# yshen47/SGAM_NeurIPS22

Hardware: AMD Instinct MI355X
Metric: generated RGB-D frames/sec (256x256, GoogleEarth) (higher is better)
Workload: dtype f32; 1 GPU; GoogleEarth-Infinite 256x256 inference loop (BASELINE configs[2]): forward-splat warp (N<=3) + VQGAN encode/quantise(4096)/decode + frame feedback, in-HBM frame store; frames_per_gpu=1110, scenes=1, parallelism=scene-parallel x1, launch=hip-graph replay of the VQGAN forward, f32_products=exact hi/lo fp16 split on the fp16 matrix cores, fp32 accumulate

## Files before the change

sgam_neurips22_amd/csrc/conv_f32x.hip:

```cpp
#include <type_traits>

#include "sgam_common.h"

namespace {

constexpr int XGN_MAXC = 1024;

typedef unsigned int u32x4 __attribute__((ext_vector_type(4)));
typedef unsigned int u32x2 __attribute__((ext_vector_type(2)));
typedef _Float16 f16x8 __attribute__((ext_vector_type(8)));

struct XParams {
    const float *x, *bias, *res;
    const unsigned short *w;
    float *out, *ws;
    int B, Hi, Wi, Cin, Ho, Wo, N, KH, KW, stride, pad_t, pad_l, ups;
    int lda, ldb, ldc, ldr, n_valid, bias_per_row;
    int M, ksplit, iters_total, iters_per_split;
    int gx, gy, xcd_swizzle;
    unsigned x_bytes, w_plane_bytes;
    const float *gn_stats, *gn_gamma, *gn_beta;
    int gn_swish;
    const double *gn_partial_in;
    double gn_inv_n;
// ... 120 lines not shown
                                           rb, (int)xsel(n < n_lim, (unsigned)n * 4u, OOB), 0, 0));
#pragma unroll
            for (int e = 0; e < 16; ++e)
                region[(i * 32 + (e & 3) + 8 * (e >> 2) + row_h) * LDR + j * 32 + col_l] = acc[i][j][e] * inv + bias_n;
        }
    constexpr int C4 = WN / 4;
    constexpr int RPP = 64 / C4;
    const int c4 = lane % C4, rr0 = lane / C4;
    const int n4 = wn0 + c4 * 4;
    const bool n_ok = n4 < n_lim;
    float gs = 0.f, gss = 0.f;
    bool bad = false;
#pragma unroll
    for (int pass = 0; pass < WM / RPP; ++pass) {
        const int row = rr0 + pass * RPP;
        const int m = rowmap(wm * (BM / WGM) + row);
        const bool ok = n_ok && m < p.M;
        f32x4 v = *reinterpret_cast<const f32x4 *>(region + row * LDR + c4 * 4);
        const f32x4 rv = __builtin_bit_cast(f32x4, __builtin_amdgcn_raw_buffer_load_b128(
                                                       rr, (int)xsel(ok, (unsigned)(m * p.ldr + n4) * 4u, OOB), 0, 0));
        if (p.bias_per_row) {
            const float bm = __builtin_bit_cast(float, __builtin_amdgcn_raw_buffer_load_b32(
                                                           rb, (int)xsel(ok, (unsigned)m * 4u, OOB), 0, 0));
            v += bm;
        }
        v += rv;
        __builtin_amdgcn_raw_buffer_store_b128(__builtin_bit_cast(u32x4, v), ro, (int)xsel(ok, (unsigned)(m * ldo + n4) * 4u, OOB), 0, 0);
        if (ok) {
            const float t4 = (v[0] + v[1]) + (v[2] + v[3]);
            gs += t4;
            gss += (v[0] * v[0] + v[1] * v[1]) + (v[2] * v[2] + v[3] * v[3]);
            bad |= sgam_not_finite(t4);
        }
    }
    if (bad && !to_ws && p.range_flag) atomicOr(p.range_flag, 1);
    if (p.gn_partial && !to_ws) {
        float *sl = region;
        sl[lane * 2] = gs;
        sl[lane * 2 + 1] = gss;
        const int c4_per_group = p.gn_cpg / 4;
        const int groups_here = C4 / c4_per_group;
        if (lane < groups_here) {
            double ds = 0.0, dss = 0.0;
            for (int r = 0; r < RPP; ++r)
                for (int k = 0; k < c4_per_group; ++k) {
                    const int l = r * C4 + lane * c4_per_group + k;
                    ds += (double)sl[l * 2];
                    dss += (double)sl[l * 2 + 1];
                }
            const int g = (wn0 / p.gn_cpg) + lane;
            const int groups = p.N / p.gn_cpg;
            if (g < groups) {
                const int chunk = bx * 2 + wm;
                const int hw = p.Ho * p.Wo;
                const int b = (bx * BM) / hw;
                const int chunks_per_b = ((hw + BM - 1) / BM) * 2;
                const int cb = chunk - b * chunks_per_b;
                double *o = p.gn_partial + (((int64_t)b * chunks_per_b + cb) * groups + g) * 2;
                o[0] = ds;
                o[1] = dss;
                if (WGM == 1) {
                    o[groups * 2] = 0.0;
                    o[groups * 2 + 1] = 0.0;
                }
            }
        }
    }
}

template <int BM, int BN, bool UPS, bool ASCALE>
__global__ __launch_bounds__(256 * wk_of(BM, BN)) void conv_gemm_f32x_kernel(const XParams p) {
    constexpr int XBK = xbk_of(BM, BN), WK = wk_of(BM, BN), NT = 256 * WK;
    constexpr int XLD = XBK + 8;
    constexpr int TM = BM / 64, TN = BN / 64;
    constexpr int PF = (BM * BN >= 128 * 128) ? 1 : 2;
    constexpr int AC = XBK / 4;
    static_assert(NT / AC == 32, "the A staging map assumes 32 rows per pass");
    constexpr int AR = BM / 32;
    constexpr int SL = XBK / 32;
    constexpr int NPB = (BN / 32) * SL * 256 / NT;
    constexpr int KS = XBK / 16;
    static_assert(KS % WK == 0, "k-steps split evenly over the wavefront groups");
    constexpr int PLANE_A = BM * XLD, PLANE_B = BN * XLD;
    constexpr int STAGE = 2 * PLANE_A + 2 * PLANE_B;
    __shared__ __attribute__((aligned(16))) unsigned short smem[2 * STAGE];

    const int tid = threadIdx.x;
    const int lane = tid & 63;
    const int wave = (tid >> 6) & 3;
    const int wk = tid >> 8;
    const int wm = wave >> 1, wn = wave & 1;
    int bx, by, bz;
    xcd_block(p, bx, by, bz);
    const int m0 = bx * BM;
    const int n0 = by * BN;

    const __amdgpu_buffer_rsrc_t rx = __builtin_amdgcn_make_buffer_rsrc((void *)p.x, 0, (int)p.x_bytes, 0x00020000);
    const __amdgpu_buffer_rsrc_t rw = __builtin_amdgcn_make_buffer_rsrc((void *)p.w, 0, (int)p.w_plane_bytes, 0x00020000);

    const int it0 = bz * p.iters_per_split;
    const int it1 = min(p.iters_total, it0 + p.iters_per_split);

    const int col4 = tid % AC;
    const int row_in_pass = tid / AC;
    const int Hl = p.ups ? 2 * p.Hi : p.Hi;
    const int Wl = p.ups ? 2 * p.Wi : p.Wi;

    int a_iy0[AR], a_ix0[AR], a_base[AR];
    unsigned a_rowoff[AR], a_tapmask[AR];
#pragma unroll
    for (int r = 0; r < AR; ++r) {
        const int m = m0 + row_in_pass + 32 * r;
        const bool ok = m < p.M;
        const int mm = ok ? m : 0;
        const int hw = p.Ho * p.Wo;
        const int b = mm / hw;
        const int rem = mm - b * hw;
        const int oy = rem / p.Wo;
        const int ox = rem - oy * p.Wo;
        a_iy0[r] = ok ? oy * p.stride - p.pad_t : -(1 << 28);
        a_ix0[r] = ox * p.stride - p.pad_l;
        a_base[r] = b * p.Hi * p.Wi;
        a_rowoff[r] = (unsigned)((a_base[r] + a_iy0[r] * p.Wi + a_ix0[r]) * p.lda + col4 * 4) * 4u;
        unsigned mk = 0;
        for (int t = 0; t < p.KH * p.KW; ++t) {
            const int iy = a_iy0[r] + t / p.KW, ix = a_ix0[r] + t % p.KW;
            mk |= (((unsigned)iy < (unsigned)p.Hi && (unsigned)ix < (unsigned)p.Wi) ? 1u : 0u) << t;
        }
        a_tapmask[r] = mk;
    }
    unsigned b_off[NPB];
    int b_lds[NPB], b_k[NPB];
    const unsigned slabs_per_row = (unsigned)p.ldb / 32u;
#pragma unroll
    for (int j = 0; j < NPB; ++j) {
        const int L = tid + NT * j, blk = L >> 8, pi = L & 255;
        const int nt = blk / SL, sl = blk - nt * SL;
        const int plane = pi >> 7, kk = (pi >> 6) & 1, kh = (pi >> 5) & 1, row = pi & 31;
        const int n = n0 + nt * 32 + row;
        b_off[j] = n < p.N ? ((((unsigned)(n >> 5) * slabs_per_row + (unsigned)sl) * 256u + (unsigned)pi) * 16u) : 0xC0000000u;
        b_lds[j] = plane * PLANE_B + (nt * 32 + row) * XLD + sl * 32 + kk * 16 + kh * 8;
        b_k[j] = sl * 32 + kk * 16 + kh * 8;
    }

    const int taps = p.KH * p.KW;
    int ch = it0 / taps;
    int tap = it0 - ch * taps;
    int ky = tap / p.KW;
    int kx = tap - ky * p.KW;

    f32x4 areg[PF][AR];
    u32x4 bp[PF][NPB];
    auto issue_loads = [&](const int st, bool live) {
        const int coff = ch * XBK + col4 * 4;
        const bool k_ok = live && coff < p.Cin;
        if constexpr (UPS) {
#pragma unroll
            for (int r = 0; r < AR; ++r) {
                const int iy = a_iy0[r] + ky, ix = a_ix0[r] + kx;
                const bool ok = k_ok && (unsigned)iy < (unsigned)Hl && (unsigned)ix < (unsigned)Wl;
                const int py = iy >> 1, px = ix >> 1;
                const unsigned off = (unsigned)((a_base[r] + py * p.Wi + px) * p.lda + coff) * 4u;
                areg[st][r] = __builtin_bit_cast(f32x4, __builtin_amdgcn_raw_buffer_load_b128(rx, (int)xsel(ok, off, p.x_bytes), 0, 0));
            }
        } else {
            const unsigned tap_off = (unsigned)((ky * p.Wi + kx) * p.lda + ch * XBK) * 4u;
#pragma unroll
            for (int r = 0; r < AR; ++r) {
                const bool ok = k_ok && ((a_tapmask[r] >> tap) & 1u);
                areg[st][r] = __builtin_bit_cast(f32x4, __builtin_amdgcn_raw_buffer_load_b128(
                                                            rx, (int)xsel(ok, a_rowoff[r] + tap_off, p.x_bytes), 0, 0));
            }
        }
        const unsigned koff = (unsigned)(tap * p.Cin + ch * XBK) * 128u;
#pragma unroll
        for (int j = 0; j < NPB; ++j) {
            const bool kb_ok = live && (ch * XBK + b_k[j]) < p.Cin;
            bp[st][j] = __builtin_amdgcn_raw_buffer_load_b128(rw, (int)xsel(kb_ok, b_off[j] + koff, p.w_plane_bytes), 0, 0);
        }
        ++tap;
        if (++kx == p.KW) {
            kx = 0;
            ++ky;
        }
        if (tap == taps) {
            tap = 0; ky = 0; kx = 0;
            ++ch;
        }
    };
    auto store_lds = [&](const int st, int buf) {
        unsigned short *ah = smem + buf * STAGE;
        unsigned short *al = ah + PLANE_A;
        unsigned short *bhp = al + PLANE_A;
#pragma unroll
        for (int r = 0; r < AR; ++r) {
            u32x2 hi, lo;
            split4(ASCALE ? areg[st][r] * p.a_scale : areg[st][r], hi, lo);
            const int o = (row_in_pass + 32 * r) * XLD + col4 * 4;
            *reinterpret_cast<u32x2 *>(ah + o) = hi;
            *reinterpret_cast<u32x2 *>(al + o) = lo;
        }
#pragma unroll
        for (int j = 0; j < NPB; ++j) *reinterpret_cast<u32x4 *>(bhp + b_lds[j]) = bp[st][j];
    };

    constexpr bool SEPACC = (TM * TN == 1);
    f32x16 acc[TM][TN], accs[1];
#pragma unroll
    for (int i = 0; i < TM; ++i)
#pragma unroll
        for (int j = 0; j < TN; ++j)
#pragma unroll
            for (int e = 0; e < 16; ++e) acc[i][j][e] = 0.f;
#pragma unroll
    for (int e = 0; e < 16; ++e) accs[0][e] = 0.f;

    const int frag_row = lane & 31;
    const int frag_k = (lane >> 5) * 8;

#pragma unroll
    for (int s = 0; s < PF; ++s) issue_loads(s, it0 + s < it1);
    store_lds(0, 0);
    issue_loads(0, it0 + PF < it1);
    __syncthreads();

    int it = it0;
    while (it < it1) {
#pragma unroll
        for (int s = 0; s < PF; ++s) {
            if (it < it1) {
                const int nst = (s + 1) % PF;
                const int buf = (it - it0) & 1;
                const unsigned short *ah = smem + buf * STAGE + (wm * (BM / 2) + frag_row) * XLD + frag_k;
                const unsigned short *al = ah + PLANE_A;
                const unsigned short *bhp = smem + buf * STAGE + 2 * PLANE_A + (wn * (BN / 2) + frag_row) * XLD + frag_k;
                const unsigned short *blp = bhp + PLANE_B;
#pragma unroll
                for (int kq = 0; kq < KS / WK; ++kq) {
                    const int kk = kq * WK + wk;
                    if (kq == (KS / WK) / 2) {
                        store_lds(nst, buf ^ 1);
                        issue_loads(nst, it + 1 + PF < it1);
                        __builtin_amdgcn_sched_barrier(0);
                    }
                    u32x4 fah[TM], fal[TM], fbh[TN], fbl[TN];
#pragma unroll
                    for (int i = 0; i < TM; ++i) {
                        fah[i] = *reinterpret_cast<const u32x4 *>(ah + i * 32 * XLD + kk * 16);
                        fal[i] = *reinterpret_cast<const u32x4 *>(al + i * 32 * XLD + kk * 16);
                    }
#pragma unroll
                    for (int j = 0; j < TN; ++j) {
                        fbh[j] = *reinterpret_cast<const u32x4 *>(bhp + j * 32 * XLD + kk * 16);
                        fbl[j] = *reinterpret_cast<const u32x4 *>(blp + j * 32 * XLD + kk * 16);
                    }
#pragma unroll
                    for (int i = 0; i < TM; ++i)
#pragma unroll
                        for (int j = 0; j < TN; ++j) {
                            if constexpr (SEPACC) {
                                accs[0] = mfma16(fal[i], fbh[j], accs[0]);
                                acc[i][j] = mfma16(fah[i], fbh[j], acc[i][j]);
                                accs[0] = mfma16(fah[i], fbl[j], accs[0]);
                            } else {
                                acc[i][j] = mfma16(fal[i], fbh[j], acc[i][j]);
                                acc[i][j] = mfma16(fah[i], fbl[j], acc[i][j]);
                                acc[i][j] = mfma16(fah[i], fbh[j], acc[i][j]);
                            }
                        }
                }
                __syncthreads();
                ++it;
            }
        }
    }

    if constexpr (SEPACC) acc[0][0] += accs[0];
    constexpr int WM = 32 * TM, WN = 32 * TN, LDR = WN + 4;
    static_assert(4 * WM * LDR * 4 <= 2 * STAGE * 2, "epilogue staging must fit the operand LDS");
    if constexpr (WK > 1) {
        constexpr int XCH = 4 * WM * LDR;
        static_assert((XCH + 4 * TM * TN * 1024) * 4 <= 2 * STAGE * 2, "k-group exchange must fit the operand LDS");
        float *xch = reinterpret_cast<float *>(smem) + XCH + wave * (TM * TN * 1024);
        if (wk == 1) {
#pragma unroll
            for (int i = 0; i < TM; ++i)
#pragma unroll
                for (int j = 0; j < TN; ++j)
#pragma unroll
                    for (int e = 0; e < 16; ++e) xch[((i * TN + j) * 16 + e) * 64 + lane] = acc[i][j][e];
        }
        __syncthreads();
        if (wk == 1) return;
#pragma unroll
        for (int i = 0; i < TM; ++i)
#pragma unroll
            for (int j = 0; j < TN; ++j)
#pragma unroll
                for (int e = 0; e < 16; ++e) acc[i][j][e] += xch[((i * TN + j) * 16 + e) * 64 + lane];
    }
    xepilogue<BM, BN, 2>(p, acc, reinterpret_cast<float *>(smem), wave, lane, bx, bz, n0, [&](int row) { return m0 + row; });
}

template <int BM, int BN, bool GN, bool UPS = false, bool GNF = false, int NB = 3>
__global__ __launch_bounds__(256, (BM == 64 && !GNF) ? XLB64 : 2) void conv3x3_f32x_halo2_kernel(const XParams p) {
    static_assert(!GNF || GN, "GNF = GroupNorm statistics folded from the producer's chunk partials: a GN kernel");
    constexpr int WGM_ = BN == 32 ? 4 : (BN == 64 ? 2 : 1), WGN_ = 4 / WGM_;
    constexpr int TH = 8, TW = BM / 8, TWS = (TW == 16) ? 4 : 3;
    constexpr int HROWS = UPS ? TH / 2 + 2 : TH + 2, HWID = UPS ? TW / 2 + 2 : TW + 2, HR = HROWS * HWID;
    static_assert(!(UPS && GN), "no GroupNorm precedes an upsampling conv");
    static_assert(BM == 128 || BM == 64, "8 x 16 or 8 x 8 output patches");
    constexpr int XBK = 32, XLD = XBK + 8;
    constexpr int TM = BM / (32 * WGM_), TN = BN / (32 * WGN_);
    constexpr int LP = UPS ? ((TW == 16) ? 408 : 240) : ((TW == 16) ? 768 : 448);
    constexpr int HPL = HROWS * LP;
    constexpr int HBUF = 2 * HPL;
    constexpr int NH = (HR * 8 + 255) / 256;
    constexpr int OP_BYTES = 2 * HBUF * 2;
    constexpr int EPI_BYTES = 4 * (32 * TM) * (32 * TN + 4) * 4;
    constexpr int TAB_BYTES = (GN && !GNF) ? XGN_MAXC * 8 : 0;
    constexpr int SM_BYTES = (OP_BYTES + TAB_BYTES) > EPI_BYTES ? (OP_BYTES + TAB_BYTES) : EPI_BYTES;
    __shared__ __attribute__((aligned(16))) unsigned short smem[SM_BYTES / 2];
    float *gn_tab = reinterpret_cast<float *>(smem + OP_BYTES / 2);

    const int tid = threadIdx.x;
    const int lane = tid & 63;
    const int wave = tid >> 6;
    const int wm = WGM_ == 4 ? wave : (WGM_ == 2 ? wave >> 1 : 0), wn = WGM_ == 4 ? 0 : (WGM_ == 2 ? (wave & 1) : wave);
    int bx, by, bz;
    xcd_block(p, bx, by, bz);
    const int n0 = by * BN;
    const int tiles_x = p.Wo / TW, tiles_img = tiles_x * (p.Ho / TH);
    const int b = bx / tiles_img;
    const int t_img = bx - b * tiles_img;
    const int ty0 = (t_img / tiles_x) * TH, tx0 = (t_img % tiles_x) * TW;

    const __amdgpu_buffer_rsrc_t rx = __builtin_amdgcn_make_buffer_rsrc((void *)p.x, 0, (int)p.x_bytes, 0x00020000);
    const __amdgpu_buffer_rsrc_t rw = __builtin_amdgcn_make_buffer_rsrc((void *)p.w, 0, (int)p.w_plane_bytes, 0x00020000);

    const int it0 = bz * p.iters_per_split;
    const int it1 = min(p.iters_total, it0 + p.iters_per_split);

    unsigned h_off[NH];
    int h_lds[NH];
#pragma unroll
    for (int j = 0; j < NH; ++j) {
        const int idx = tid + 256 * j;
        const int row = idx >> 3, col4 = idx & 7;
        const int hy = row / HWID, hx = row - hy * HWID;
        const int iy = (UPS ? ty0 / 2 : ty0) + hy - 1, ix = (UPS ? tx0 / 2 : tx0) + hx - 1;
        const bool ok = row < HR && (unsigned)iy < (unsigned)p.Hi && (unsigned)ix < (unsigned)p.Wi;
        h_off[j] = ok ? (unsigned)(((b * p.Hi + iy) * p.Wi + ix) * p.lda + col4 * 4) * 4u : 0xFFFFFFFFu;
        h_lds[j] = row < HR ? hy * LP + hx * XLD + col4 * 4 : -1;
    }
    unsigned bf_off[TN];
#pragma unroll
    for (int j = 0; j < TN; ++j) {
        const int nt = (n0 + wn * (BN / WGN_) + j * 32) >> 5;
        bf_off[j] = ((unsigned)nt * ((unsigned)p.ldb / 32u) * 256u + (unsigned)lane) * 16u;
    }

    f32x4 hreg[NH];
    f32x4 gt0, gt1;
    auto hload_issue = [&](int ch, bool live) {
        const unsigned coff = (unsigned)ch * (XBK * 4u);
#pragma unroll
        for (int j = 0; j < NH; ++j)
            hreg[j] = __builtin_bit_cast(f32x4, __builtin_amdgcn_raw_buffer_load_b128(rx, (int)(live ? h_off[j] : 0xFFFFFFFFu), (int)coff, 0));
    };
    auto hparams = [&](int ch, bool live) {
        if constexpr (GN && GNF) {
            gn_scale_shift<GNF>(p, b, (live ? ch : 0) * XBK + (tid & 7) * 4, gt0, gt1);
        } else if constexpr (GN) {
            const float *t = gn_tab + 2 * ((live ? ch : 0) * XBK + (tid & 7) * 4);
            gt0 = *reinterpret_cast<const f32x4 *>(t);
            gt1 = *reinterpret_cast<const f32x4 *>(t + 4);
        }
    };
    auto hload = [&](int ch, bool live) {
        hload_issue(ch, live);
        hparams(ch, live);
    };
    auto hprep_piece = [&](const int j) {
        {
            u32x2 hi, lo;
            f32x4 v = hreg[j];
            if constexpr (GN) {
                v[0] = v[0] * gt0[0] + gt0[1];
                v[1] = v[1] * gt0[2] + gt0[3];
                v[2] = v[2] * gt1[0] + gt1[1];
                v[3] = v[3] * gt1[2] + gt1[3];
                if (p.gn_swish) {
#pragma unroll
                    for (int e = 0; e < 4; ++e) v[e] = sgam_swish(v[e]);
                }
                if (h_off[j] == 0xFFFFFFFFu) v = f32x4{0.f, 0.f, 0.f, 0.f};
            }
            split4(v, hi, lo);
            hreg[j] = __builtin_bit_cast(f32x4, u32x4{hi[0], hi[1], lo[0], lo[1]});
        }
    };
    auto hprep = [&]() {
#pragma unroll
        for (int j = 0; j < NH; ++j) hprep_piece(j);
    };
    auto hstore = [&](int hb) {
        unsigned short *halo = smem + hb * HBUF;
#pragma unroll
        for (int j = 0; j < NH; ++j) {
            const u32x4 q = __builtin_bit_cast(u32x4, hreg[j]);
            if (h_lds[j] >= 0) {
                *reinterpret_cast<u32x2 *>(halo + h_lds[j]) = u32x2{q[0], q[1]};
                *reinterpret_cast<u32x2 *>(halo + HPL + h_lds[j]) = u32x2{q[2], q[3]};
            }
        }
    };

    static_assert(NB == 3 || NB == 6, "ring of three or of six");
    u32x4 bq[NB][TN][2][2];
    auto bload = [&](const int set, int tap, int ch, bool live) {
        const unsigned koff = (unsigned)(tap * p.Cin + ch * XBK) * 128u;
#pragma unroll
        for (int j = 0; j < TN; ++j) {
            const unsigned vo = live ? bf_off[j] : 0xFFFFFFF0u;
#pragma unroll
            for (int kk = 0; kk < 2; ++kk)
#pragma unroll
                for (int pl = 0; pl < 2; ++pl)
                    bq[set][j][kk][pl] = __builtin_amdgcn_raw_buffer_load_b128(rw, (int)vo, (int)(koff + (unsigned)((pl * 2 + kk) * 1024)), 0);
        }
    };

    f32x16 acc[TM][TN];
#pragma unroll
    for (int i = 0; i < TM; ++i)
#pragma unroll
        for (int j = 0; j < TN; ++j)
#pragma unroll
            for (int e = 0; e < 16; ++e) acc[i][j][e] = 0.f;

    const int frag_row = lane & 31;
    const int frag_k = (lane >> 5) * 8;
    int a_base[TM], a_py[TM], a_px[TM];
#pragma unroll
    for (int i = 0; i < TM; ++i) {
        const int r = wm * (BM / WGM_) + i * 32 + frag_row;
        a_py[i] = r >> TWS;
        a_px[i] = r & (TW - 1);
        a_base[i] = a_py[i] * LP + a_px[i] * XLD + frag_k;
    }

    const int s0 = it0 / 9, s1 = it1 / 9;
    int hcur = 0;
    hload_issue(s0, s0 < s1);
#pragma unroll
    for (int t = 0; t < NB - 1; ++t) bload(t, t, s0, s0 < s1);
    if constexpr (GN && !GNF) {
        const int cpg = p.Cin / 32;
        constexpr int CPT = XGN_MAXC / 256;
        float mr[CPT][2];
#pragma unroll
        for (int k = 0; k < CPT; ++k) {
            const int c = tid + 256 * k;
            if (c < p.Cin) mr[k][0] = p.gn_stats[(b * 32 + c / cpg) * 2], mr[k][1] = p.gn_stats[(b * 32 + c / cpg) * 2 + 1];
        }
#pragma unroll
        for (int k = 0; k < CPT; ++k) {
            const int c = tid + 256 * k;
            if (c < p.Cin) {
                const float sc = mr[k][1] * p.gn_gamma[c];
                gn_tab[2 * c] = sc;
                gn_tab[2 * c + 1] = p.gn_beta[c] - mr[k][0] * sc;
            }
        }
        __syncthreads();
    }
    hparams(s0, s0 < s1);
    hprep();
    hstore(0);
    if (s0 + 1 < s1) hload(s0 + 1, true);
    __syncthreads();

    u32x4 fa[2][TM][2];
    const unsigned short *hb = smem;
    auto afrag = [&](const int set, const int tap, const int kk) {
        const int ky = tap / 3, kx = tap - 3 * ky;
#pragma unroll
        for (int i = 0; i < TM; ++i) {
            const unsigned short *ah;
            if constexpr (UPS) ah = hb + (((a_py[i] + ky - 1) >> 1) + 1) * LP + (((a_px[i] + kx - 1) >> 1) + 1) * XLD + frag_k;
            else ah = hb + ky * LP + kx * XLD + a_base[i];
            fa[set][i][0] = *reinterpret_cast<const u32x4 *>(ah + kk * 16);
            fa[set][i][1] = *reinterpret_cast<const u32x4 *>(ah + HPL + kk * 16);
        }
    };
#define XDS_READ(dst, addr, off) asm volatile("ds_read_b128 %0, %1 offset:%2" : "=v"(dst) : "v"(addr), "i"(off))
    unsigned a_lds[TM];
    auto afrag_asm = [&](const int set, const int tap, const int kk) {
        const int ky = tap / 3, kx = tap - 3 * ky;
#pragma unroll
        for (int i = 0; i < TM; ++i) {
            XDS_READ(fa[set][i][0], a_lds[i], 2 * (ky * LP + kx * XLD + kk * 16));
            XDS_READ(fa[set][i][1], a_lds[i], 2 * (ky * LP + kx * XLD + kk * 16 + HPL));
        }
    };
    auto await = [&](const int set, const bool next_in_flight) {
        if constexpr (TM == 4) {
            if (next_in_flight)
                asm volatile("s_waitcnt lgkmcnt(8)" : "+v"(fa[set][0][0]), "+v"(fa[set][0][1]), "+v"(fa[set][1][0]), "+v"(fa[set][1][1]),
                             "+v"(fa[set][2][0]), "+v"(fa[set][2][1]), "+v"(fa[set][3][0]), "+v"(fa[set][3][1]));
            else
                asm volatile("s_waitcnt lgkmcnt(0)" : "+v"(fa[set][0][0]), "+v"(fa[set][0][1]), "+v"(fa[set][1][0]), "+v"(fa[set][1][1]),
                             "+v"(fa[set][2][0]), "+v"(fa[set][2][1]), "+v"(fa[set][3][0]), "+v"(fa[set][3][1]));
        } else if constexpr (TM == 2) {
            if (next_in_flight)
                asm volatile("s_waitcnt lgkmcnt(4)" : "+v"(fa[set][0][0]), "+v"(fa[set][0][1]), "+v"(fa[set][1][0]), "+v"(fa[set][1][1]));
            else
                asm volatile("s_waitcnt lgkmcnt(0)" : "+v"(fa[set][0][0]), "+v"(fa[set][0][1]), "+v"(fa[set][1][0]), "+v"(fa[set][1][1]));
        } else {
            static_assert(TM == 1 || TM == 2 || TM == 4, "wait counts are spelled for 1, 2 or 4 row tiles");
            if (next_in_flight) asm volatile("s_waitcnt lgkmcnt(2)" : "+v"(fa[set][0][0]), "+v"(fa[set][0][1]));
            else asm volatile("s_waitcnt lgkmcnt(0)" : "+v"(fa[set][0][0]), "+v"(fa[set][0][1]));
        }
    };
    constexpr bool XASM = !UPS;
    auto slab = [&](const int sl, auto mode_, auto rb_) {
        constexpr int MODE = decltype(mode_)::value, RB = decltype(rb_)::value;
        const bool has_next = MODE != 3;
        const bool has_next2 = MODE == 1;
        hb = smem + hcur * HBUF;
        if constexpr (XASM) {
            const unsigned hb_lds = (unsigned)(uintptr_t)(__attribute__((address_space(3))) const unsigned short *)hb;
#pragma unroll
            for (int i = 0; i < TM; ++i) a_lds[i] = hb_lds + 2u * (unsigned)a_base[i];
        }
#pragma unroll
        for (int tap = 0; tap < 9; ++tap) {
            const int set = (tap + RB) % NB;
            const int tt = tap + NB - 1;
            if (tt < 9) bload((tt + RB) % NB, tt, sl, true);
            else if constexpr (MODE != 3) bload((tt + RB) % NB, tt - 9, sl + 1, has_next);
            if constexpr (MODE != 3) {
                if (tap >= 1 && tap <= NH) hprep_piece(tap - 1);
                if (tap == NH + 1) {
                    hstore(hcur ^ 1);
                    if constexpr (MODE != 2) hload(sl + 2, has_next2);
                }
            }
#pragma unroll
            for (int kk = 0; kk < 2; ++kk) {
                const int q = tap * 2 + kk;
                if constexpr (XASM) {
                    if (q == 0) afrag_asm(0, 0, 0);
                    if (q < 17) afrag_asm((q + 1) & 1, (q + 1) >> 1, (q + 1) & 1);
                    await(q & 1, q < 17);
                } else {
                    if (q == 0) afrag(0, 0, 0);
                    if (q < 17) afrag((q + 1) & 1, (q + 1) >> 1, (q + 1) & 1);
                }
#pragma unroll
                for (int term = 0; term < 3; ++term)
#pragma unroll
                    for (int i = 0; i < TM; ++i)
#pragma unroll
                        for (int j = 0; j < TN; ++j) {
                            acc[i][j] = mfma16(fa[q & 1][i][term == 0 ? 1 : 0], bq[set][j][kk][term == 1 ? 1 : 0], acc[i][j]);
                        }
            }
        }
        __syncthreads();
        hcur ^= 1;
    };
    typedef std::integral_constant<int, 0> I0;
    typedef std::integral_constant<int, 1> I1;
    typedef std::integral_constant<int, 2> I2;
    typedef std::integral_constant<int, 3> I3;
    if constexpr (NB == 3) {
        if (s0 < s1) {
            int sl = s0;
            for (; sl + 2 < s1; ++sl) slab(sl, I1{}, I0{});
            if (s1 - s0 >= 2) slab(s1 - 2, I2{}, I0{});
            slab(s1 - 1, I3{}, I0{});
        }
    } else if constexpr (GNF) {
        if (s1 - s0 >= 2) {
            slab(s0, I2{}, I0{});
            slab(s0 + 1, I3{}, I3{});
        } else if (s0 < s1) {
            slab(s0, I3{}, I0{});
        }
    } else if (s0 < s1) {
        int sl = s0;
        for (; sl + 2 < s1; sl += 2) {
            slab(sl, I1{}, I0{});
            slab(sl + 1, I1{}, I3{});
        }
        slab(s1 - 2, I2{}, I0{});
        slab(s1 - 1, I3{}, I3{});
    }
    __syncthreads();

    xepilogue<BM, BN, WGM_>(p, acc, reinterpret_cast<float *>(smem), wave, lane, bx, bz, n0, [&](int row) {
        return (b * p.Ho + ty0 + (row >> TWS)) * p.Wo + tx0 + (row & (TW - 1));
    });
}


__global__ __launch_bounds__(256) void splitk_reduce_f32x_kernel(const XParams p) {
    const int64_t q = (int64_t)blockIdx.x * blockDim.x + threadIdx.x;
    const int nq = p.N / 4;
    const bool live = q < (int64_t)p.M * nq;
    const int m = live ? (int)(q / nq) : 0;
    const int n = live ? (int)(q - (int64_t)m * nq) * 4 : 0;
    float gs = 0.f, gss = 0.f;
    if (live) {
        const float *w0 = p.ws + (int64_t)m * p.N + n;
        const int64_t zs = (int64_t)p.M * p.N;
        float bv[4], rv[4];
#pragma unroll
        for (int e = 0; e < 4; ++e) {
            const bool ok = n + e < p.n_valid;
            bv[e] = (ok && p.bias) ? (p.bias_per_row ? p.bias[m] : p.bias[n + e]) : 0.f;
            rv[e] = (ok && p.res) ? p.res[(int64_t)m * p.ldr + n + e] : 0.f;
        }
        f32x4 s = *reinterpret_cast<const f32x4 *>(w0);
        int z = 1;
        for (; z + 4 <= p.ksplit; z += 4) {
            const f32x4 a = *reinterpret_cast<const f32x4 *>(w0 + z * zs), b = *reinterpret_cast<const f32x4 *>(w0 + (z + 1) * zs);
            const f32x4 c = *reinterpret_cast<const f32x4 *>(w0 + (z + 2) * zs), d = *reinterpret_cast<const f32x4 *>(w0 + (z + 3) * zs);
            s += a;
            s += b;
            s += c;
            s += d;
        }
        for (; z < p.ksplit; ++z) s += *reinterpret_cast<const f32x4 *>(w0 + z * zs);
#pragma unroll
        for (int e = 0; e < 4; ++e) {
            if (n + e >= p.n_valid) continue;
            float v = s[e] * p.inv_w_scale;
            if (p.bias) v += bv[e];
            if (p.res) v += rv[e];
            p.out[(int64_t)m * p.ldc + n + e] = v;
            gs += v;
            gss += v * v;
        }
        if (p.range_flag && sgam_not_finite(gs)) atomicOr(p.range_flag, 1);
    }
    if (!p.gn_partial) return;
    const int c4n = p.gn_cpg / 4;
    for (int o = 1; o < c4n; o <<= 1) {
        gs += __shfl_xor(gs, o, 64);
        gss += __shfl_xor(gss, o, 64);
    }
    __shared__ float sh[8][32][2];
    const int rows = 1024 / p.N, row = threadIdx.x / nq, g = (threadIdx.x - row * nq) / c4n;
    if ((threadIdx.x % c4n) == 0) {
        sh[row][g][0] = gs;
        sh[row][g][1] = gss;
    }
    __syncthreads();
    if (threadIdx.x < 32) {
        double ds = 0.0, dss = 0.0;
        for (int r = 0; r < rows; ++r) {
            ds += (double)sh[r][threadIdx.x][0];
            dss += (double)sh[r][threadIdx.x][1];
        }
        double *o = p.gn_partial + ((int64_t)blockIdx.x * 32 + threadIdx.x) * 2;
        o[0] = ds;
        o[1] = dss;
    }
}

template <int TC>
__global__ __launch_bounds__(256) void splitk_reduce_gm_f32x_kernel(const XParams p) {
    constexpr int TR = 1024 / TC, TPR = TC / 4;
    const int col_tiles = p.N / TC;
    const int rt = blockIdx.x / col_tiles, ct = blockIdx.x - rt * col_tiles;
    const int row = threadIdx.x / TPR, c4 = threadIdx.x - row * TPR;
    const int m = rt * TR + row, n = ct * TC + c4 * 4;
    const float *w0 = p.ws + (int64_t)m * p.N + n;
    const int64_t zs = (int64_t)p.M * p.N;
    f32x4 bv = {0.f, 0.f, 0.f, 0.f}, rv = {0.f, 0.f, 0.f, 0.f};
    if (p.bias) bv = p.bias_per_row ? f32x4{p.bias[m], p.bias[m], p.bias[m], p.bias[m]} : *reinterpret_cast<const f32x4 *>(p.bias + n);
    if (p.res) rv = *reinterpret_cast<const f32x4 *>(p.res + (int64_t)m * p.ldr + n);
    f32x4 s = *reinterpret_cast<const f32x4 *>(w0);
    int z = 1;
    for (; z + 4 <= p.ksplit; z += 4) {
        const f32x4 a = *reinterpret_cast<const f32x4 *>(w0 + z * zs), b = *reinterpret_cast<const f32x4 *>(w0 + (z + 1) * zs);
        const f32x4 c = *reinterpret_cast<const f32x4 *>(w0 + (z + 2) * zs), d = *reinterpret_cast<const f32x4 *>(w0 + (z + 3) * zs);
        s += a;
        s += b;
        s += c;
        s += d;
    }
    for (; z < p.ksplit; ++z) s += *reinterpret_cast<const f32x4 *>(w0 + z * zs);
    f32x4 v;
#pragma unroll
    for (int e = 0; e < 4; ++e) {
        v[e] = s[e] * p.inv_w_scale;
        if (p.bias) v[e] += bv[e];
        if (p.res) v[e] += rv[e];
    }
    *reinterpret_cast<f32x4 *>(p.out + (int64_t)m * p.ldc + n) = v;
    float gs = (v[0] + v[1]) + (v[2] + v[3]);
    float gss = (v[0] * v[0] + v[1] * v[1]) + (v[2] * v[2] + v[3] * v[3]);
    if (p.range_flag && sgam_not_finite(gs)) atomicOr(p.range_flag, 1);
    if (!p.gn_partial) return;
    const int lpg = p.gn_cpg / 4;
    for (int o = 1; o < lpg; o <<= 1) {
        gs += __shfl_xor(gs, o, 64);
        gss += __shfl_xor(gss, o, 64);
    }
    __shared__ float sh[256][2];
    const int gt = TC / p.gn_cpg, gl = c4 / lpg;
    if ((c4 % lpg) == 0) {
        sh[row * gt + gl][0] = gs;
        sh[row * gt + gl][1] = gss;
    }
    __syncthreads();
    if ((int)threadIdx.x < gt) {
        double ds = 0.0, dss = 0.0;
        for (int r = 0; r < TR; ++r) {
            ds += (double)sh[r * gt + threadIdx.x][0];
            dss += (double)sh[r * gt + threadIdx.x][1];
        }
        double *o = p.gn_partial + ((int64_t)rt * 32 + ct * gt + threadIdx.x) * 2;
        o[0] = ds;
        o[1] = dss;
    }
}

__device__ __forceinline__ int64_t frag_index(int64_t n, int64_t k, int64_t slabs_per_row) {
    const int64_t slab = k >> 5, kin = k & 31;
    const int64_t piece = (((kin >> 4) * 2) + ((kin >> 3) & 1)) * 32 + (n & 31);
    return (((n >> 5) * slabs_per_row + slab) * 256 + piece) * 8 + (kin & 7);
}

__global__ void pack_weight_f32x_kernel(const float *w, unsigned short *o, int Cout, int Cin, int KH, int KW, int Cout_pad,
                                        int Cin_pad, float scale) {
    const int64_t i = (int64_t)blockIdx.x * blockDim.x + threadIdx.x;
    const int taps = KH * KW;
    const int64_t total = (int64_t)Cout_pad * taps * Cin_pad;
    if (i >= total) return;
    const int c = (int)(i % Cin_pad);
    const int t = (int)((i / Cin_pad) % taps);
    const int n = (int)(i / ((int64_t)Cin_pad * taps));
    float v = 0.f;
    if (n < Cout && c < Cin) v = w[((int64_t)n * Cin + c) * taps + t] * scale;
    const _Float16 h = (_Float16)v;
    const _Float16 l = (_Float16)(v - (float)h);
    const int64_t k = (int64_t)t * Cin_pad + c;
    const int64_t q = frag_index(n, k, (int64_t)taps * Cin_pad / 32);
    o[q] = __builtin_bit_cast(unsigned short, h);
    o[q + 2 * 2 * 32 * 8] = __builtin_bit_cast(unsigned short, l);
}

__global__ void split_rows_f32x_kernel(const float *x, unsigned short *o, int N, int Np, int K, int Kp, int ld, float scale) {
    const int64_t i = (int64_t)blockIdx.x * blockDim.x + threadIdx.x;
    const int64_t total = (int64_t)Np * Kp;
    if (i >= total) return;
    const int n = (int)(i / Kp), k = (int)(i - (int64_t)n * Kp);
    const float v = (k < K && n < N) ? x[(int64_t)n * ld + k] * scale : 0.f;
    const _Float16 h = (_Float16)v;
    const _Float16 l = (_Float16)(v - (float)h);
    const int64_t q = frag_index(n, k, Kp / 32);
    o[q] = __builtin_bit_cast(unsigned short, h);
    o[q + 2 * 2 * 32 * 8] = __builtin_bit_cast(unsigned short, l);
}

struct XPlan {
    int bm, bn, ksplit, iters_total, iters_per_split;
};

static bool halo_shape(const sgam_conv_desc *d, int bm, int bn) {
    const bool tile_ok = (bm == 128 && bn == 128 && d->Wo % 16 == 0) || (bm == 64 && bn == 128 && d->Wo % 8 == 0) ||
                         (bm == 128 && bn == 32 && d->Wo % 16 == 0 && d->N == 32 && !d->upsample2x) ||
                         (bm == 64 && bn == 64 && d->Wo % 8 == 0 && d->N % 64 == 0 && !d->upsample2x);
    const int up = d->upsample2x ? 2 : 1;
    return tile_ok && d->KH == 3 && d->KW == 3 && d->stride == 1 && d->pad_t == 1 && d->pad_l == 1 &&
           d->Ho == up * d->Hi && d->Wo == up * d->Wi && d->Ho % 8 == 0 && d->Cin % 32 == 0;
}

XPlan make_xplan(const sgam_conv_desc *d) {
    const int64_t M = (int64_t)d->B * d->Ho * d->Wo;
    XPlan pl;
    auto blocks = [&](int bm, int bn) { return (int64_t)sgam_cdiv(M, bm) * sgam_cdiv(d->N, bn); };
    if (d->N == 32 && d->plan_bm == 0 && halo_shape(d, 128, 32)) { pl.bm = 128; pl.bn = 32; }
    else if (d->N % 128 == 0 && blocks(128, 128) >= 224) { pl.bm = 128; pl.bn = 128; }
    else if (d->N % 128 == 0 && blocks(64, 128) >= 224) { pl.bm = 64; pl.bn = 128; }
    else { pl.bm = 64; pl.bn = 64; }
    if (d->plan_bm > 0 && d->plan_bn > 0) { pl.bm = d->plan_bm; pl.bn = d->plan_bn; }
    const int xbk = halo_shape(d, pl.bm, pl.bn) ? 32 : xbk_of(pl.bm, pl.bn);
    pl.iters_total = d->KH * d->KW * ((d->Cin + xbk - 1) / xbk);
    const int64_t nb = blocks(pl.bm, pl.bn);
    int ks = 1;
    if (d->plan_ksplit > 0) {
        ks = d->plan_ksplit;
        if (ks > pl.iters_total) ks = pl.iters_total;
    } else if (nb < 192) {
        ks = (int)((384 + nb - 1) / nb);
        const int max_by_iters = pl.iters_total / 4;
        if (ks > max_by_iters) ks = max_by_iters;
        if (ks > 32) ks = 32;
        if (ks < 1) ks = 1;
    }
    pl.iters_per_split = (pl.iters_total + ks - 1) / ks;
    if (halo_shape(d, pl.bm, pl.bn)) pl.iters_per_split = (pl.iters_per_split + 8) / 9 * 9;
    pl.ksplit = (pl.iters_total + pl.iters_per_split - 1) / pl.iters_per_split;
    return pl;
}

int xvalidate(const sgam_conv_desc *d) {
    if (!d) return SGAM_EINVAL;
    if (d->B <= 0 || d->Hi <= 0 || d->Wi <= 0 || d->Ho <= 0 || d->Wo <= 0 || d->N <= 0) return SGAM_EINVAL;
    if (d->Cin <= 0 || d->Cin % 8 != 0 || d->N % 4 != 0) return SGAM_EINVAL;
    if (d->KH <= 0 || d->KW <= 0 || d->stride <= 0) return SGAM_EINVAL;
    if (d->lda < d->Cin || d->lda % 4 != 0) return SGAM_EALIGN;
    if (d->ldb < d->KH * d->KW * d->Cin || d->ldb % 32 != 0) return SGAM_EALIGN;
    if (d->KH * d->KW > 1 && d->Cin % 32 != 0) return SGAM_EALIGN;
    if (d->n_valid <= 0 || d->n_valid > d->N || d->ldc < d->n_valid) return SGAM_EINVAL;
    if (d->n_valid % 4 != 0 || d->ldc % 4 != 0 || d->ldr % 4 != 0) return SGAM_EALIGN;
    if (d->plan_bm != 0 || d->plan_bn != 0) {
        const bool ok = (d->plan_bm == 128 && d->plan_bn == 128) || (d->plan_bm == 64 && d->plan_bn == 128) ||
                        (d->plan_bm == 128 && d->plan_bn == 32 && d->N == 32) ||
                        (d->plan_bm == 64 && d->plan_bn == 64);
        if (!ok || (d->plan_bn == 128 && d->N % 128 != 0)) return SGAM_EINVAL;
    }
    if (d->plan_ksplit < 0 || d->plan_ksplit > 64) return SGAM_EINVAL;
    return SGAM_OK;
}

}

extern "C" int64_t sgam_conv2d_f32x_workspace_bytes(const sgam_conv_desc *d) {
    if (xvalidate(d) != SGAM_OK) return -1;
    const XPlan pl = make_xplan(d);
    if (pl.ksplit <= 1) return 0;
    return (int64_t)pl.ksplit * d->B * d->Ho * d->Wo * d->N * (int64_t)sizeof(float);
}

extern "C" int sgam_conv2d_f32x_plan(const sgam_conv_desc *d, int32_t *bm, int32_t *bn, int32_t *ksplit) {
    const int rc = xvalidate(d);
    if (rc != SGAM_OK) return rc;
    const XPlan pl = make_xplan(d);
    if (bm) *bm = pl.bm;
    if (bn) *bn = pl.bn;
    if (ksplit) *ksplit = pl.ksplit;
    return SGAM_OK;
}

struct XExtra {
    const float *gn_stats = nullptr, *gn_gamma = nullptr, *gn_beta = nullptr;
    int gn_swish = 0;
    const double *gn_partial_in = nullptr;
    int gn_chunks_in = 0;
    float gn_eps = 1e-6f;
    double *gn_partial = nullptr;
};

static int conv_f32x_impl(const sgam_conv_desc *d, const float *x, float a_scale, const void *w_planes, float w_scale,
                          const float *bias, const float *residual, float *out, void *workspace, int64_t workspace_bytes,
                          void *stream, const XExtra &ex);

static bool halo_eligible(const sgam_conv_desc *d, const XPlan &pl, float a_scale) {
    return a_scale == 1.0f && halo_shape(d, pl.bm, pl.bn);
}

extern "C" int32_t sgam_conv2d_f32x_uses_halo(const sgam_conv_desc *d) {
    if (xvalidate(d) != SGAM_OK) return 0;
    return halo_eligible(d, make_xplan(d), 1.0f) ? 1 : 0;
}

extern "C" int32_t sgam_conv2d_f32x_gn_fusable(const sgam_conv_desc *d) {
    if (xvalidate(d) != SGAM_OK || d->upsample2x || d->Cin > XGN_MAXC) return 0;
    return halo_eligible(d, make_xplan(d), 1.0f) ? 1 : 0;
}

static int red_tc_for(const sgam_conv_desc *d) {
    const int hw = d->Ho * d->Wo, cpg = d->N / 32;
    if (d->N % 128 != 0 || d->n_valid != d->N || d->N > 1024) return 0;
    for (int tc = 32; tc >= 8; tc >>= 1) {
        const int tr = 1024 / tc;
        if (tc >= cpg && tc % cpg == 0 && (cpg & (cpg - 1)) == 0 && hw % tr == 0 && hw / tr <= 16) return tc;
    }
    return 0;
}

extern "C" int32_t sgam_conv2d_f32x_stats_chunks(const sgam_conv_desc *d) {
    if (xvalidate(d) != SGAM_OK) return -1;
    const XPlan pl = make_xplan(d);
    const int hw = d->Ho * d->Wo;
    if (d->N % 128 != 0 || d->n_valid != d->N) return 0;
    if (pl.ksplit == 1) {
        if (d->B > 1 && hw % pl.bm != 0) return 0;
        return ((hw + pl.bm - 1) / pl.bm) * 2;
    }
    if (const int tc = red_tc_for(d)) return hw / (1024 / tc);
    if (d->N > 1024 || 1024 % d->N != 0 || ((int64_t)hw * d->N) % 1024 != 0) return 0;
    return (int32_t)((int64_t)hw * d->N / 1024);
}

extern "C" int32_t sgam_conv2d_f32x_stats_mode(const sgam_conv_desc *d) {
    return sgam_conv2d_f32x_stats_chunks(d) > 0 ? 1 : 0;
}

static int check_stats_out(const sgam_conv_desc *d, const XExtra &ex) {
    return (ex.gn_partial && sgam_conv2d_f32x_stats_mode(d) != 1) ? SGAM_EINVAL : SGAM_OK;
}

extern "C" int sgam_conv2d_gn_nhwc_f32x(const sgam_conv_desc *d, const float *x, const float *gn_mean_rstd, const float *gn_gamma,
                                        const float *gn_beta, int32_t gn_swish, const void *w_planes, float w_scale,
                                        const float *bias, const float *residual, float *out, double *gn_partial,
                                        void *workspace, int64_t workspace_bytes, void *stream) {
    if (!gn_mean_rstd || !gn_gamma || !gn_beta || !sgam_aligned16(gn_gamma) || !sgam_aligned16(gn_beta) ||
        sgam_conv2d_f32x_gn_fusable(d) != 1 || d->Cin % 128 != 0)
        return SGAM_EINVAL;
    XExtra ex;
    ex.gn_stats = gn_mean_rstd; ex.gn_gamma = gn_gamma; ex.gn_beta = gn_beta; ex.gn_swish = gn_swish ? 1 : 0;
    ex.gn_partial = gn_partial;
    if (check_stats_out(d, ex) != SGAM_OK) return SGAM_EINVAL;
    return conv_f32x_impl(d, x, 1.0f, w_planes, w_scale, bias, residual, out, workspace, workspace_bytes, stream, ex);
}

extern "C" int32_t sgam_conv2d_f32x_gn_foldable(const sgam_conv_desc *d, int32_t chunks_in) {
    if (chunks_in < 1 || chunks_in > 16 || sgam_conv2d_f32x_gn_fusable(d) != 1 || d->Cin % 128 != 0) return 0;
    const XPlan pl = make_xplan(d);
    return (pl.bm == 64 && pl.bn == 128 && pl.iters_per_split <= 18) ? 1 : 0;
}

extern "C" int sgam_conv2d_gnp_nhwc_f32x(const sgam_conv_desc *d, const float *x, const double *gn_partial_in, int32_t chunks_in,
                                         float eps, const float *gn_gamma, const float *gn_beta, int32_t gn_swish, const void *w_planes,
                                         float w_scale, const float *bias, const float *residual, float *out, double *gn_partial,
                                         void *workspace, int64_t workspace_bytes, void *stream) {
    if (!gn_partial_in || !gn_gamma || !gn_beta || !sgam_aligned16(gn_partial_in) || !sgam_aligned16(gn_gamma) ||
        !sgam_aligned16(gn_beta) || !(eps > 0.f) || sgam_conv2d_f32x_gn_foldable(d, chunks_in) != 1)
        return SGAM_EINVAL;
    XExtra ex;
    ex.gn_partial_in = gn_partial_in;
    ex.gn_chunks_in = chunks_in; ex.gn_eps = eps;
    ex.gn_gamma = gn_gamma; ex.gn_beta = gn_beta; ex.gn_swish = gn_swish ? 1 : 0;
    ex.gn_partial = gn_partial;
    if (check_stats_out(d, ex) != SGAM_OK) return SGAM_EINVAL;
    return conv_f32x_impl(d, x, 1.0f, w_planes, w_scale, bias, residual, out, workspace, workspace_bytes, stream, ex);
}

extern "C" int sgam_conv2d_nhwc_f32x(const sgam_conv_desc *d, const float *x, float a_scale, const void *w_planes,
                                     float w_scale, const float *bias, const float *residual, float *out,
                                     void *workspace, int64_t workspace_bytes, void *stream) {
    return conv_f32x_impl(d, x, a_scale, w_planes, w_scale, bias, residual, out, workspace, workspace_bytes, stream, XExtra());
}

extern "C" int sgam_conv2d_stats_nhwc_f32x(const sgam_conv_desc *d, const float *x, float a_scale, const void *w_planes,
                                           float w_scale, const float *bias, const float *residual, float *out,
                                           double *gn_partial, void *workspace, int64_t workspace_bytes, void *stream) {
    XExtra ex;
    ex.gn_partial = gn_partial;
    if (!gn_partial || check_stats_out(d, ex) != SGAM_OK) return SGAM_EINVAL;
    return conv_f32x_impl(d, x, a_scale, w_planes, w_scale, bias, residual, out, workspace, workspace_bytes, stream, ex);
}

static int conv_f32x_impl(const sgam_conv_desc *d, const float *x, float a_scale, const void *w_planes, float w_scale,
                          const float *bias, const float *residual, float *out, void *workspace, int64_t workspace_bytes,
                          void *stream, const XExtra &ex) {
    const int rc = xvalidate(d);
    if (rc != SGAM_OK) return rc;
    if (!x || !w_planes || !out || !(w_scale > 0.f) || !(a_scale > 0.f)) return SGAM_EINVAL;
    if (!sgam_aligned16(x) || !sgam_aligned16(w_planes)) return SGAM_EALIGN;
    const XPlan pl = make_xplan(d);
    XParams p;
    p.x = x; p.w = (const unsigned short *)w_planes; p.bias = bias; p.res = residual; p.out = out; p.ws = nullptr;
    p.B = d->B; p.Hi = d->Hi; p.Wi = d->Wi; p.Cin = d->Cin; p.Ho = d->Ho; p.Wo = d->Wo; p.N = d->N;
    p.KH = d->KH; p.KW = d->KW; p.stride = d->stride; p.pad_t = d->pad_t; p.pad_l = d->pad_l; p.ups = d->upsample2x ? 1 : 0;
    p.lda = d->lda; p.ldb = d->ldb; p.ldc = d->ldc; p.ldr = d->ldr; p.n_valid = d->n_valid; p.bias_per_row = d->bias_per_row;
    p.M = d->B * d->Ho * d->Wo;
    p.ksplit = pl.ksplit; p.iters_total = pl.iters_total; p.iters_per_split = pl.iters_per_split;
    p.inv_w_scale = 1.0f / (w_scale * a_scale);
    p.range_flag = sgam_i_range_flag;
    p.a_scale = a_scale;
    p.gn_partial = ex.gn_partial;
    p.gn_cpg = d->N / 32;
    p.gn_stats = ex.gn_stats; p.gn_gamma = ex.gn_gamma; p.gn_beta = ex.gn_beta;
    p.gn_swish = ex.gn_swish;
    p.gn_partial_in = ex.gn_partial_in; p.gn_chunks_in = ex.gn_chunks_in; p.gn_eps = ex.gn_eps;
    p.gn_inv_n = 1.0 / ((double)d->Hi * d->Wi * (d->Cin / 32));
    p.red_tc = 0;

    const int64_t xb = (((int64_t)d->B * d->Hi * d->Wi - 1) * d->lda + d->Cin) * 4;
    const int64_t wb = (int64_t)((d->N + 31) / 32 * 32) * d->ldb * 4;
    if (xb >= (1ll << 32) - 64 || wb >= (1ll << 32) - 256) return SGAM_EINVAL;
    p.x_bytes = (unsigned)xb; p.w_plane_bytes = (unsigned)wb;
    if (pl.ksplit > 1) {
        const int64_t need = (int64_t)pl.ksplit * p.M * p.N * (int64_t)sizeof(float);
        if (!workspace || workspace_bytes < need || !sgam_aligned16(workspace)) return SGAM_EWORKSPACE;
        p.ws = (float *)workspace;
    }
    p.gx = sgam_cdiv(p.M, pl.bm);
    p.gy = sgam_cdiv(p.N, pl.bn);
    p.xcd_swizzle = 1;
    const dim3 grid((unsigned)((int64_t)p.gx * p.gy * pl.ksplit));
    hipStream_t s = sgam_stream(stream);
#define XLAUNCH(BM_, BN_)                                                                                                   \
    do {                                                                                                                    \
        const dim3 blk(256 * wk_of(BM_, BN_));                                                                              \
        if (p.ups) SGAM_KLAUNCH((conv_gemm_f32x_kernel<BM_, BN_, true, false>), grid, blk, 0, s, p);                  \
        else if (a_scale != 1.0f) SGAM_KLAUNCH((conv_gemm_f32x_kernel<BM_, BN_, false, true>), grid, blk, 0, s, p);   \
        else SGAM_KLAUNCH((conv_gemm_f32x_kernel<BM_, BN_, false, false>), grid, blk, 0, s, p);                       \
    } while (0)
    if (p.ups && a_scale != 1.0f) return SGAM_EINVAL;
    if (d->KH * d->KW > 32) return SGAM_EINVAL;
    const bool halo = halo_eligible(d, pl, a_scale);
    const bool gn_tab_on = ex.gn_stats != nullptr;
    if ((gn_tab_on || ex.gn_partial_in) && !halo) return SGAM_EINVAL;
    if (gn_tab_on && d->Cin > XGN_MAXC) return SGAM_EINVAL;
    if (ex.gn_partial_in && (pl.bm != 64 || p.ups)) return SGAM_EINVAL;
    if (sgam_i_prof_on) sgam_i_prof_shape(p.M, d->n_valid, d->KH * d->KW * d->Cin, pl.ksplit);
    if (sgam_i_prof_on)
        sgam_i_prof_work(2.0 * p.M * d->n_valid * (double)(d->KH * d->KW * d->Cin),
                         4.0 * ((double)d->B * d->Hi * d->Wi * d->Cin + (double)d->n_valid * d->KH * d->KW * d->Cin +
                                (double)p.M * d->n_valid * (residual ? 2 : 1)));
    if (halo) {
        if (p.ups) {
            if (pl.bm == 128) SGAM_KLAUNCH((conv3x3_f32x_halo2_kernel<128, 128, false, true>), grid, dim3(256), 0, s, p);
            else SGAM_KLAUNCH((conv3x3_f32x_halo2_kernel<64, 128, false, true>), grid, dim3(256), 0, s, p);
        } else if (pl.bm == 128 && pl.bn == 32) {
            if (gn_tab_on) SGAM_KLAUNCH((conv3x3_f32x_halo2_kernel<128, 32, true>), grid, dim3(256), 0, s, p);
            else SGAM_KLAUNCH((conv3x3_f32x_halo2_kernel<128, 32, false>), grid, dim3(256), 0, s, p);
        } else if (pl.bm == 128) {
            if (gn_tab_on) SGAM_KLAUNCH((conv3x3_f32x_halo2_kernel<128, 128, true>), grid, dim3(256), 0, s, p);
            else SGAM_KLAUNCH((conv3x3_f32x_halo2_kernel<128, 128, false>), grid, dim3(256), 0, s, p);
        } else if (pl.bn == 64) {
            if (p.gn_partial_in) return SGAM_EINVAL;
            if (gn_tab_on) SGAM_KLAUNCH((conv3x3_f32x_halo2_kernel<64, 64, true>), grid, dim3(256), 0, s, p);
            else SGAM_KLAUNCH((conv3x3_f32x_halo2_kernel<64, 64, false>), grid, dim3(256), 0, s, p);
        } else {
            const int slabs_wg = p.iters_per_split / 9;
            const bool deep6 = (int64_t)grid.x * grid.y * grid.z <= 2 * 256 && p.iters_per_split % 9 == 0 &&
                               (p.gn_partial_in ? slabs_wg <= 2 : (slabs_wg % 2 == 0 && (p.iters_total / 9) % slabs_wg == 0));
            if (deep6 && p.gn_partial_in) SGAM_KLAUNCH((conv3x3_f32x_halo2_kernel<64, 128, true, false, true, 6>), grid, dim3(256), 0, s, p);
            else if (deep6 && gn_tab_on) SGAM_KLAUNCH((conv3x3_f32x_halo2_kernel<64, 128, true, false, false, 6>), grid, dim3(256), 0, s, p);
            else if (p.gn_partial_in) SGAM_KLAUNCH((conv3x3_f32x_halo2_kernel<64, 128, true, false, true>), grid, dim3(256), 0, s, p);
            else if (gn_tab_on) SGAM_KLAUNCH((conv3x3_f32x_halo2_kernel<64, 128, true>), grid, dim3(256), 0, s, p);
            else SGAM_KLAUNCH((conv3x3_f32x_halo2_kernel<64, 128, false>), grid, dim3(256), 0, s, p);
        }
    } else if (pl.bm == 128 && pl.bn == 128) XLAUNCH(128, 128);
    else if (pl.bm == 64 && pl.bn == 128) XLAUNCH(64, 128);
    else XLAUNCH(64, 64);
#undef XLAUNCH
    SGAM_LAUNCH_CHECK();
    if (pl.ksplit > 1) {
        const int64_t q = (int64_t)p.M * (p.N / 4);
        const int tc = p.gn_partial ? red_tc_for(d) : 0;
        if (tc == 32) SGAM_KLAUNCH(splitk_reduce_gm_f32x_kernel<32>, dim3((unsigned)(q / 256)), dim3(256), 0, s, p);
        else if (tc == 16) SGAM_KLAUNCH(splitk_reduce_gm_f32x_kernel<16>, dim3((unsigned)(q / 256)), dim3(256), 0, s, p);
        else if (tc == 8) SGAM_KLAUNCH(splitk_reduce_gm_f32x_kernel<8>, dim3((unsigned)(q / 256)), dim3(256), 0, s, p);
        else SGAM_KLAUNCH(splitk_reduce_f32x_kernel, dim3(sgam_cdiv(q, 256)), dim3(256), 0, s, p);
        SGAM_LAUNCH_CHECK();
    }
    return SGAM_OK;
}

extern "C" int sgam_pack_conv_weight_f32x(const float *w_oihw, void *w_planes, float w_scale, int32_t Cout, int32_t Cin,
                                          int32_t KH, int32_t KW, int32_t Cout_pad, int32_t Cin_pad, void *stream) {
    if (!w_oihw || !w_planes || Cout <= 0 || Cin <= 0 || KH <= 0 || KW <= 0 || Cout_pad < Cout || Cin_pad < Cin || Cin_pad % 32 || Cout_pad % 32) return SGAM_EINVAL;
    const int64_t total = (int64_t)Cout_pad * KH * KW * Cin_pad;
    SGAM_KLAUNCH(pack_weight_f32x_kernel, dim3(sgam_cdiv(total, 256)), dim3(256), 0, sgam_stream(stream), w_oihw,
                       (unsigned short *)w_planes, Cout, Cin, KH, KW, Cout_pad, Cin_pad, w_scale);
    SGAM_LAUNCH_CHECK();
    return SGAM_OK;
}

extern "C" int sgam_split_rows_f32x(const float *x, void *planes, float scale, int32_t N, int32_t K, int32_t ld, void *stream) {
    if (!x || !planes || N <= 0 || K <= 0 || ld < K) return SGAM_EINVAL;
    const int Kp = (K + 31) / 32 * 32, Np = (N + 31) / 32 * 32;
    const int64_t total = (int64_t)Np * Kp;
    SGAM_KLAUNCH(split_rows_f32x_kernel, dim3(sgam_cdiv(total, 256)), dim3(256), 0, sgam_stream(stream), x,
                       (unsigned short *)planes, N, Np, K, Kp, ld, scale);
    SGAM_LAUNCH_CHECK();
    return SGAM_OK;
}

extern "C" int sgam_debug_f32x_occupancy(int which) {
    int n = -1;
    hipError_t e;
    if (which == 0) e = hipOccupancyMaxActiveBlocksPerMultiprocessor(&n, conv_gemm_f32x_kernel<128, 128, false, false>, 256, 0);
    else if (which == 1) e = hipOccupancyMaxActiveBlocksPerMultiprocessor(&n, conv_gemm_f32x_kernel<64, 128, false, false>, 256, 0);
    else e = hipOccupancyMaxActiveBlocksPerMultiprocessor(&n, conv_gemm_f32x_kernel<64, 64, false, false>, 256 * wk_of(64, 64), 0);
    return e == hipSuccess ? n : -(int)e;
}
```

Baseline: 371.8 frames/s.

## Use a four-slot weight ring with split halo prefetch for 128-row halo convs

For 128-row halo 3x3 conv tiles, the fixed three-slot rotating weight prefetch ring becomes a four-slot ring driven by a hand-built tap-to-slot schedule. That schedule issues some weight loads two or more taps ahead. The next slab's halo load is split into two halves, loaded, prepped and stored at different taps, with sched_barriers added. The goal is to hide global-load latency and spread halo register pressure across the slab, at the cost of more live registers and a more fragile schedule.

```diff
diff --git a/sgam_neurips22_amd/csrc/conv_f32x.hip b/sgam_neurips22_amd/csrc/conv_f32x.hip
--- a/sgam_neurips22_amd/csrc/conv_f32x.hip
+++ b/sgam_neurips22_amd/csrc/conv_f32x.hip
@@ -446,6 +446,15 @@
     xepilogue<BM, BN, 2>(p, acc, reinterpret_cast<float *>(smem), wave, lane, bx, bz, n0, [&](int row) { return m0 + row; });
 }
 
+__host__ __device__ constexpr int ring4_set(int tap) {
+    constexpr int s[9] = {0, 1, 2, 3, 0, 2, 3, 1, 2};
+    return s[tap];
+}
+__host__ __device__ constexpr int ring4_request(int tap, int k) {
+    constexpr int r[9][2] = {{2, 3}, {-1, -1}, {4, -1}, {5, -1}, {6, 7}, {-1, -1}, {8, -1}, {9, -1}, {10, -1}};
+    return r[tap][k];
+}
+
 template <int BM, int BN, bool GN, bool UPS = false, bool GNF = false, int NB = 3>
 __global__ __launch_bounds__(256, (BM == 64 && !GNF) ? XLB64 : 2) void conv3x3_f32x_halo2_kernel(const XParams p) {
     static_assert(!GNF || GN, "GNF = GroupNorm statistics folded from the producer's chunk partials: a GN kernel");
@@ -525,6 +534,12 @@
         hload_issue(ch, live);
         hparams(ch, live);
     };
+    auto hload_part = [&](int ch, const int j0, const int j1) {
+        const unsigned coff = (unsigned)ch * (XBK * 4u);
+#pragma unroll
+        for (int j = j0; j < j1; ++j)
+            hreg[j] = __builtin_bit_cast(f32x4, __builtin_amdgcn_raw_buffer_load_b128(rx, (int)h_off[j], (int)coff, 0));
+    };
     auto hprep_piece = [&](const int j) {
         {
             u32x2 hi, lo;
@@ -548,10 +563,10 @@
 #pragma unroll
         for (int j = 0; j < NH; ++j) hprep_piece(j);
     };
-    auto hstore = [&](int hb) {
+    auto hstore_part = [&](int hb, const int j0, const int j1) {
         unsigned short *halo = smem + hb * HBUF;
 #pragma unroll
-        for (int j = 0; j < NH; ++j) {
+        for (int j = j0; j < j1; ++j) {
             const u32x4 q = __builtin_bit_cast(u32x4, hreg[j]);
             if (h_lds[j] >= 0) {
                 *reinterpret_cast<u32x2 *>(halo + h_lds[j]) = u32x2{q[0], q[1]};
@@ -559,8 +574,12 @@
             }
         }
     };
-
-    static_assert(NB == 3 || NB == 6, "ring of three or of six");
+    auto hstore = [&](int hb) { hstore_part(hb, 0, NH); };
+
+    static_assert(NB == 3 || NB == 4 || NB == 6, "ring of three, four or six");
+    static_assert(NB != 4 || (BM == 128 && !GNF), "the ring of four is the 128-row tile's");
+    constexpr bool HSPLIT = NB == 4;
+    constexpr int NHA = (NH + 1) / 2;
     u32x4 bq[NB][TN][2][2];
     auto bload = [&](const int set, int tap, int ch, bool live) {
         const unsigned koff = (unsigned)(tap * p.Cin + ch * XBK) * 128u;
@@ -598,7 +617,7 @@
     int hcur = 0;
     hload_issue(s0, s0 < s1);
 #pragma unroll
-    for (int t = 0; t < NB - 1; ++t) bload(t, t, s0, s0 < s1);
+    for (int t = 0; t < (HSPLIT ? 2 : NB - 1); ++t) bload(t, t, s0, s0 < s1);
     if constexpr (GN && !GNF) {
         const int cpg = p.Cin / 32;
         constexpr int CPT = XGN_MAXC / 256;
@@ -622,7 +641,9 @@
     hparams(s0, s0 < s1);
     hprep();
     hstore(0);
-    if (s0 + 1 < s1) hload(s0 + 1, true);
+    if constexpr (!HSPLIT) {
+        if (s0 + 1 < s1) hload(s0 + 1, true);
+    }
     __syncthreads();
 
     u32x4 fa[2][TM][2];
@@ -680,11 +701,43 @@
         }
 #pragma unroll
         for (int tap = 0; tap < 9; ++tap) {
-            const int set = (tap + RB) % NB;
+            const int set = HSPLIT ? ring4_set(tap) : (tap + RB) % NB;
             const int tt = tap + NB - 1;
-            if (tt < 9) bload((tt + RB) % NB, tt, sl, true);
-            else if constexpr (MODE != 3) bload((tt + RB) % NB, tt - 9, sl + 1, has_next);
-            if constexpr (MODE != 3) {
+            if constexpr (HSPLIT) __builtin_amdgcn_sched_barrier(0);
+            if constexpr (HSPLIT) {
+#pragma unroll
+                for (int k = 0; k < 2; ++k) {
+                    const int t4 = ring4_request(tap, k);
+                    if (t4 >= 0 && t4 < 9) bload(ring4_set(t4), t4, sl, true);
+                    else if constexpr (MODE != 3) {
+                        if (t4 >= 9) bload(ring4_set(t4 - 9), t4 - 9, sl + 1, true);
+                    }
+                }
+            } else {
+                if (tt < 9) bload((tt + RB) % NB, tt, sl, true);
+                else if constexpr (MODE != 3) bload((tt + RB) % NB, tt - 9, sl + 1, has_next);
+            }
+            if constexpr (HSPLIT) {
+                if constexpr (MODE != 3) {
+                    if (tap == 0) {
+                        hparams(sl + 1, true);
+                        hload_part(sl + 1, 0, NHA);
+                    }
+                    if (tap == 3 && NHA > 1) hprep_piece(0);
+                    if (tap == 4) {
+#pragma unroll
+                        for (int j = NHA > 1 ? 1 : 0; j < NHA; ++j) hprep_piece(j);
+                        hstore_part(hcur ^ 1, 0, NHA);
+                        hload_part(sl + 1, NHA, NH);
+                    }
+                    if (tap == 7 && NH - NHA > 1) hprep_piece(NHA);
+                    if (tap == 8) {
+#pragma unroll
+                        for (int j = NH - NHA > 1 ? NHA + 1 : NHA; j < NH; ++j) hprep_piece(j);
+                        hstore_part(hcur ^ 1, NHA, NH);
+                    }
+                }
+            } else if constexpr (MODE != 3) {
                 if (tap >= 1 && tap <= NH) hprep_piece(tap - 1);
                 if (tap == NH + 1) {
                     hstore(hcur ^ 1);
@@ -719,7 +772,13 @@
     typedef std::integral_constant<int, 1> I1;
     typedef std::integral_constant<int, 2> I2;
     typedef std::integral_constant<int, 3> I3;
-    if constexpr (NB == 3) {
+    if constexpr (NB == 4) {
+        if (s0 < s1) {
+            int sl = s0;
+            for (; sl + 1 < s1; ++sl) slab(sl, I1{}, I0{});
+            slab(s1 - 1, I3{}, I0{});
+        }
+    } else if constexpr (NB == 3) {
         if (s0 < s1) {
             int sl = s0;
             for (; sl + 2 < s1; ++sl) slab(sl, I1{}, I0{});
@@ -1164,14 +1223,14 @@
                                 (double)p.M * d->n_valid * (residual ? 2 : 1)));
     if (halo) {
         if (p.ups) {
-            if (pl.bm == 128) SGAM_KLAUNCH((conv3x3_f32x_halo2_kernel<128, 128, false, true>), grid, dim3(256), 0, s, p);
+            if (pl.bm == 128) SGAM_KLAUNCH((conv3x3_f32x_halo2_kernel<128, 128, false, true, false, 4>), grid, dim3(256), 0, s, p);
             else SGAM_KLAUNCH((conv3x3_f32x_halo2_kernel<64, 128, false, true>), grid, dim3(256), 0, s, p);
         } else if (pl.bm == 128 && pl.bn == 32) {
-            if (gn_tab_on) SGAM_KLAUNCH((conv3x3_f32x_halo2_kernel<128, 32, true>), grid, dim3(256), 0, s, p);
-            else SGAM_KLAUNCH((conv3x3_f32x_halo2_kernel<128, 32, false>), grid, dim3(256), 0, s, p);
+            if (gn_tab_on) SGAM_KLAUNCH((conv3x3_f32x_halo2_kernel<128, 32, true, false, false, 4>), grid, dim3(256), 0, s, p);
+            else SGAM_KLAUNCH((conv3x3_f32x_halo2_kernel<128, 32, false, false, false, 4>), grid, dim3(256), 0, s, p);
         } else if (pl.bm == 128) {
-            if (gn_tab_on) SGAM_KLAUNCH((conv3x3_f32x_halo2_kernel<128, 128, true>), grid, dim3(256), 0, s, p);
-            else SGAM_KLAUNCH((conv3x3_f32x_halo2_kernel<128, 128, false>), grid, dim3(256), 0, s, p);
+            if (gn_tab_on) SGAM_KLAUNCH((conv3x3_f32x_halo2_kernel<128, 128, true, false, false, 4>), grid, dim3(256), 0, s, p);
+            else SGAM_KLAUNCH((conv3x3_f32x_halo2_kernel<128, 128, false, false, false, 4>), grid, dim3(256), 0, s, p);
         } else if (pl.bn == 64) {
             if (p.gn_partial_in) return SGAM_EINVAL;
             if (gn_tab_on) SGAM_KLAUNCH((conv3x3_f32x_halo2_kernel<64, 64, true>), grid, dim3(256), 0, s, p);
```

After: 370.8 frames/s. No clear change (-0.3%).
